# wushan270/mit-6.824-2015

Hardware: AMD Instinct MI355X
Metric: word-count input GB/s (whole node) and % of HBM roofline at 1/2/4/8 MI355X (higher is better)
Workload: dtype u8

## Files before the change

mit-6.824-2015_amd/csrc/wcg_agg.h:

```cpp
#pragma once
#include "wcg_common.h"
#include "wcg_lds_table.h"
#include "wcg_map.h"

namespace wcg {

constexpr int AGG_NT = 1024;
constexpr u32 AGG_BATCH = AGG_NT * 4;
constexpr int AGG_W = 2;
constexpr int AGG_NB = 3350;
constexpr u32 AGG_SLACK_UNITS = AGG_BATCH + 8;
constexpr u32 AGG_MAX_SRC = 256;
constexpr u32 AGG_Q = 128;
constexpr u32 AGG_OVF_CAP = 4096;
constexpr int AGG_SPILL = 0, AGG_EMIT = 1;
#ifndef WCG_AGG_PROBES
#define WCG_AGG_PROBES 2
#endif
constexpr int AGG_PROBES = WCG_AGG_PROBES;
#ifndef WCG_AGG_SPEC_K1
#define WCG_AGG_SPEC_K1 0
#endif
constexpr bool AGG_SPEC_K1 = WCG_AGG_SPEC_K1;
#ifndef WCG_AGG_SPEC_MED
#define WCG_AGG_SPEC_MED 1
#endif
#ifndef WCG_AGG_KINDS
#define WCG_AGG_KINDS 1
#endif
#ifndef WCG_AGG_ABLATE
#define WCG_AGG_ABLATE 0
#endif

struct AggArgs {
    const u64* pool;
    const u32* region_len;
    u64 region_cap;
    u32 P;
    u32 nsrc;
    u32 slices;
    u32 pm;
    u32 slices_m;
    u32 nbi;
    u32 ls_nreg;
    u32 rstride, rmod;
    u32 P1;
    int mode;
    GEntry* gtab;
    u64 gmask;
    DevState* st;
    const u64* map_stats;
    u64* spill;
    u64 spill_cap;
    u32* spill_len;
    Rec* emit;
    u64 emit_cap;
    Rec* ovf;
    u32 ovf_cap;
    u64* clk;
    uint16_t* flist;
};

#ifndef WCG_AGG2_LDSHASH
#define WCG_AGG2_LDSHASH 0
#endif
__device__ __forceinline__ u32 agg_hash(u64 k0, u64 k1) {
    if (WCG_AGG2_LDSHASH) return lds_hash(k0, k1) * 0x9E3779B1u;
    return (u32)(key_hash(k0, k1) >> 32);
}

__device__ __forceinline__ void agg_decode(const u64 (&u)[6], u64 (&k0)[4], u64 (&k1)[4], u64 (&c)[4], bool (&v)[4],
                                           u32 (&nu)[4]) {
#pragma unroll
    for (int k = 0; k < 4; k++) {
        const u32 T = (u32)(u[k] >> 56);
        const bool head = T >= 0x41;
        v[k] = T != 0 && (head || (T & 0x1F) < 8);
        const u64 last = head ? u[k + 1] : u[k];
        k0[k] = head ? u[k] : (u[k] & ~U_CNT);
        k1[k] = head ? (u[k + 1] & ~U_CNT) : 0;
        const bool hc = (last & U_CNT) != 0;
        c[k] = hc ? (head ? u[k + 2] : u[k + 1]) : 1;
        nu[k] = (head ? 2u : 1u) + (hc ? 1u : 0u);
    }
}

__device__ __forceinline__ void agg_decode_short(const u64 (&u)[6], u64 (&k0)[4], u64 (&k1)[4], u64 (&c)[4], bool (&v)[4],
                                                 u32 (&nu)[4]) {
#pragma unroll
    for (int k = 0; k < 4; k++) {
        v[k] = (u[k] >> 56) != 0;
        const bool hc = (u[k] & U_CNT) != 0;
        k0[k] = u[k] & ~U_CNT;
        k1[k] = 0;
        c[k] = hc ? u[k + 1] : 1;
        nu[k] = hc ? 2u : 1u;
    }
}
__device__ __forceinline__ void agg_decode_medium(const u64 (&u)[6], u64 (&k0)[4], u64 (&k1)[4], u64 (&c)[4], bool (&v)[4],
                                                  u32 (&nu)[4]) {
#pragma unroll
    for (int k = 0; k < 4; k++) {
        v[k] = (u32)(u[k] >> 56) >= 0x41;
        const bool hc = (u[k + 1] & U_CNT) != 0;
        k0[k] = u[k];
        k1[k] = u[k + 1] & ~U_CNT;
        c[k] = hc ? u[k + 2] : 1;
        nu[k] = hc ? 3u : 2u;
    }
}

#define WCG_AGG_SET_OPS(S)                                                                      \
    __device__ __forceinline__ void agg_load_##S(const v4u* q, v4u& x0, v4u& x1, v4u& x2) {     \
        asm volatile("global_load_dwordx4 %0, %3, off ; wcg-load " #S "0\n\t"                   \
                     "global_load_dwordx4 %1, %3, off offset:16 ; wcg-load " #S "1\n\t"         \
                     "global_load_dwordx4 %2, %3, off offset:32 ; wcg-load " #S "2"              \
                     : "=&v"(x0), "=&v"(x1), "=&v"(x2) : "v"(q) : "memory");                    \
    }                                                                                           \
    template <int N>                                                                            \
    __device__ __forceinline__ void agg_wait_##S(v4u& x0, v4u& x1, v4u& x2) {                   \
        asm volatile("s_waitcnt vmcnt(%3) ; wcg-wait " #S " %0 %1 %2"                            \
                     : "+v"(x0), "+v"(x1), "+v"(x2) : "n"(N) : "memory");                       \
    }
WCG_AGG_SET_OPS(A)
WCG_AGG_SET_OPS(B)
WCG_AGG_SET_OPS(C)
#undef WCG_AGG_SET_OPS
#ifndef WCG_AGG_SETS1
#define WCG_AGG_SETS1 2
#endif
#ifndef WCG_AGG_SETS2
#define WCG_AGG_SETS2 2
#endif

template <int MODE, int KIND>
__device__ __forceinline__ u64 agg_one(const AggArgs& a, u32 bi, u64 (*tk0)[AGG_W], u64 (*tk1)[AGG_W], u64 (*tcnt)[AGG_W], u32* rlen_s,
                       u32* bstart, u32& spos, u64 (*wsum)[4]) {
    const int tid = threadIdx.x;
    LdsTable<AGG_NB, u64, AGG_W> tab{tk0, tk1, tcnt};
    constexpr bool emit = MODE == AGG_EMIT;
    u32 p, s, sl;
    if (bi < a.pm * a.slices) { p = bi % a.pm; s = bi / a.pm; sl = a.slices; }
    else { const u32 b2 = bi - a.pm * a.slices, nm = a.P - a.pm; p = a.pm + b2 % nm; s = b2 / nm; sl = a.slices_m; }
#ifdef WCG_AGG_MREV
    if (p >= a.pm && a.pm < a.P) p = a.P - 1 - (p - a.pm);
#endif
    u32 k0_, k1_, wbase, wstep;
    if (!emit) {
        k0_ = (u32)(((u64)a.nsrc * s) / sl); k1_ = (u32)(((u64)a.nsrc * (s + 1)) / sl);
        wbase = 0; wstep = 1;
    } else {
        k0_ = 0; k1_ = a.nsrc;
        wbase = p / AGG_Q; wstep = a.P1;
    }
    const u32 nk = k1_ - k0_;
    auto region = [&](u32 k) -> u64 { return (u64)(wbase + k * wstep) * a.rstride + p % a.rmod; };
    constexpr u32 WB = 256;
    for (u32 k = tid; k < nk; k += AGG_NT) rlen_s[k] = a.region_len[region(k0_ + k)];
    __syncthreads();
    if (tid == 0) {
        u32 t = 0;
        for (u32 k = 0; k < nk; k++) { bstart[k] = t; t += (rlen_s[k] + WB - 1) / WB; }
        bstart[nk] = t;
        spos = 0;
    }
    __syncthreads();
    const u32 nbat = bstart[nk];
    if (nbat == 0) {
        if (!emit && tid == 0 && a.spill_len) a.spill_len[bi] = 0;
        return 0;
    }
    tab.init(tid, AGG_NT);
    __syncthreads();
    u64 my_global = 0;
    u64* const sp = emit ? nullptr : a.spill + (u64)bi * a.spill_cap;
    auto overflow = [&](u64 k0, u64 k1, u64 c, u32 nu) {
        if (emit) {
            const u32 pos = atomicAdd(&spos, 1u);
            if (pos < a.ovf_cap) { a.ovf[(u64)blockIdx.x * a.ovf_cap + pos] = inline_rec(k0, k1, c); return; }
        } else {
            const u32 pos = atomicAdd(&spos, nu);
            if (pos + nu <= a.spill_cap) {
                u64 e[3];
                const u64 f = c > 1 ? U_CNT : 0;
                if (key_short(k0)) { e[0] = k0 | f; e[1] = c; }
                else { e[0] = k0; e[1] = k1 | f; e[2] = c; }
                for (u32 j = 0; j < nu; j++) sp[pos + j] = e[j];
                return;
            }
            for (u64 j = pos; j < a.spill_cap; j++) sp[j] = 0;
        }
        my_global++;
        ginsert(a.gtab, a.gmask, k0, k1, gslot(key_hash(k0, k1)), c, a.st);
    };
    const u32 wave = (u32)__builtin_amdgcn_readfirstlane(tid >> 6), lane = tid & 63;
    constexpr u32 WSTRIDE = AGG_NT / 64;
    const bool per_wave = !emit;
    auto advance = [&](u32& k, u32& b, u32 step) {
        if (per_wave) {
            b += step / WSTRIDE;
            while (k < nk && b >= bstart[k + 1] - bstart[k]) { k += WSTRIDE; b = 0; }
            return;
        }
        b += step;
        while (k < nk) {
            const u32 nbk = bstart[k + 1] - bstart[k];
            if (b < nbk) break;
            b -= nbk;
            k++;
        }
    };
    auto batch_ptr = [&](u32 k, u32 b) -> const v4u* {
        const bool live = k < nk;
        const u64 i = (live ? (u64)b * WB : 0) + 4 * lane;
        return reinterpret_cast<const v4u*>(a.pool + region(k0_ + (live ? k : 0)) * a.region_cap + i);
    };
    auto unit = [](const v4u& x, int h) -> u64 { return h ? ((u64)x.w << 32 | x.z) : ((u64)x.y << 32 | x.x); };
    auto process = [&](u32 k, u32 b, const v4u& x0, const v4u& x1, const v4u& x2) {
        u64 u[6] = {unit(x0, 0), unit(x0, 1), unit(x1, 0), unit(x1, 1), unit(x2, 0), unit(x2, 1)};
        const u32 i0 = b * WB + 4 * lane, len = rlen_s[k];
#pragma unroll
        for (int j = 0; j < 6; j++) u[j] = i0 + j < len ? u[j] : 0;
        if (WCG_AGG_ABLATE == 1) { asm volatile("" ::"v"(u[0] ^ u[1] ^ u[2] ^ u[3] ^ u[4] ^ u[5])); return; }
        u64 k0[4], k1[4], c[4];
        bool v[4];
        u32 nu[4];
        if (KIND == 1) agg_decode_short(u, k0, k1, c, v, nu);
        else if (KIND == 2) agg_decode_medium(u, k0, k1, c, v, nu);
        else agg_decode(u, k0, k1, c, v, nu);
        if (WCG_AGG_ABLATE == 4) {
#pragma unroll
            for (int j = 0; j < 4; j++) v[j] = v[j] && key_short(k0[j]);
        }
        if (WCG_AGG_ABLATE == 2) {
            u32 x = 0;
#pragma unroll
            for (int j = 0; j < 4; j++) x ^= v[j] ? lds_hash(k0[j], k1[j]) + (u32)c[j] : 0u;
            asm volatile("" ::"v"(x));
            return;
        }
        static_assert(4 % AGG_PROBES == 0, "probe groups split a lane's 4 units");
        constexpr bool SPEC = KIND == 2 ? WCG_AGG_SPEC_MED : AGG_SPEC_K1;
#pragma unroll
        for (int j = 0; j < 4; j += AGG_PROBES) {
            typename decltype(tab)::Probe pr[AGG_PROBES];
#pragma unroll
            for (int q = 0; q < AGG_PROBES; q++) {
                const u32 h = emit ? agg_hash(k0[j + q], k1[j + q]) : lds_hash(k0[j + q], k1[j + q]);
                if (!v[j + q]) continue;
                if (SPEC) tab.start_k1(h, KIND == 2 || !key_short(k0[j + q]), pr[q]);
                else tab.start(h, pr[q]);
            }
#pragma unroll
            for (int q = 0; q < AGG_PROBES; q++) {
                if (!v[j + q]) continue;
                const bool ok = SPEC ? tab.template finish_k1<KIND>(k0[j + q], k1[j + q], pr[q], c[j + q])
                                     : tab.template finish<KIND>(k0[j + q], k1[j + q], pr[q], c[j + q]);
                if (!ok) overflow(k0[j + q], k1[j + q], c[j + q], nu[j + q]);
            }
        }
    };
    constexpr int NSETS = emit ? WCG_AGG_SETS2 : WCG_AGG_SETS1;
    static_assert(NSETS == 2 || NSETS == 3, "k_agg's batch walk names two or three register sets");
    u32 kA = 0, bA = 0, kB, bB, kC = 0, bC = 0;
    if (per_wave) { kA = wave; bA = (u32)-1; advance(kA, bA, WSTRIDE); }
    else advance(kA, bA, wave);
    kB = kA; bB = bA;
    advance(kB, bB, WSTRIDE);
    v4u a0, a1, a2, b0, b1, b2, c0, c1, c2;
    agg_load_A(batch_ptr(kA, bA), a0, a1, a2);
    agg_load_B(batch_ptr(kB, bB), b0, b1, b2);
    if (NSETS == 3) {
        kC = kB; bC = bB;
        advance(kC, bC, WSTRIDE);
        agg_load_C(batch_ptr(kC, bC), c0, c1, c2);
        while (kA < nk) {
            agg_wait_A<6>(a0, a1, a2);
            process(kA, bA, a0, a1, a2);
            kA = kC; bA = bC;
            advance(kA, bA, WSTRIDE);
            agg_load_A(batch_ptr(kA, bA), a0, a1, a2);
            if (kB >= nk) break;
            agg_wait_B<6>(b0, b1, b2);
            process(kB, bB, b0, b1, b2);
            kB = kA; bB = bA;
            advance(kB, bB, WSTRIDE);
            agg_load_B(batch_ptr(kB, bB), b0, b1, b2);
            if (kC >= nk) break;
            agg_wait_C<6>(c0, c1, c2);
            process(kC, bC, c0, c1, c2);
            kC = kB; bC = bB;
            advance(kC, bC, WSTRIDE);
            agg_load_C(batch_ptr(kC, bC), c0, c1, c2);
        }
        agg_wait_C<0>(c0, c1, c2);
    } else {
        while (kA < nk) {
            agg_wait_A<3>(a0, a1, a2);
            process(kA, bA, a0, a1, a2);
            kA = kB; bA = bB;
            advance(kA, bA, WSTRIDE);
            agg_load_A(batch_ptr(kA, bA), a0, a1, a2);
            if (kB >= nk) break;
            agg_wait_B<3>(b0, b1, b2);
            process(kB, bB, b0, b1, b2);
            kB = kA; bB = bA;
            advance(kB, bB, WSTRIDE);
            agg_load_B(batch_ptr(kB, bB), b0, b1, b2);
        }
    }
    agg_wait_A<0>(a0, a1, a2);
    agg_wait_B<0>(b0, b1, b2);
    __syncthreads();
    if (!emit && a.flist && !a.spill_cap && WCG_AGG_ABLATE != 3) {
        constexpr u32 NE = AGG_NB * AGG_W;
        uint16_t* const L = a.flist + (u64)bi * NE;
        u32 mine = 0;
        for (int i = tid; i < (int)NE; i += AGG_NT) mine += (&tcnt[0][0])[i] ? 1u : 0u;
        u32 incl = mine;
        for (int d = 1; d < 64; d <<= 1) { const u32 y = __shfl_up(incl, d, 64); if (lane >= (u32)d) incl += y; }
        if (lane == 63) wsum[wave][0] = incl;
        __syncthreads();
        u32 pos = 0, all = 0;
        for (u32 w = 0; w < AGG_NT / 64; w++) { if (w < wave) pos += (u32)wsum[w][0]; all += (u32)wsum[w][0]; }
        pos += incl - mine;
        for (int i = tid; i < (int)NE; i += AGG_NT)
            if ((&tcnt[0][0])[i]) L[pos++] = (uint16_t)i;
        asm volatile("s_waitcnt vmcnt(0)" ::: "memory");
        __syncthreads();
        for (u32 j = tid; j < all; j += AGG_NT) {
            const u32 i = __hip_atomic_load(&L[j], __ATOMIC_RELAXED, __HIP_MEMORY_SCOPE_AGENT);
            const u64 c = (&tcnt[0][0])[i], k0 = (&tk0[0][0])[i], k1 = (&tk1[0][0])[i];
            my_global++;
            ginsert(a.gtab, a.gmask, k0, k1, gslot(key_hash(k0, k1)), c, a.st);
        }
        __syncthreads();
    } else if (!emit) {
        for (int i = tid; i < AGG_NB * AGG_W; i += AGG_NT) {
            const u64 c = (&tcnt[0][0])[i];
            if (!c || WCG_AGG_ABLATE == 3) continue;
            const u64 k0 = (&tk0[0][0])[i], k1 = (&tk1[0][0])[i];
            if (a.spill_cap) { overflow(k0, k1, c, (u32)entry_units(k0, (u32)(c > 1 ? 2 : 1))); continue; }
            my_global++;
            ginsert(a.gtab, a.gmask, k0, k1, gslot(key_hash(k0, k1)), c, a.st);
        }
        __syncthreads();
        if (tid == 0 && a.spill_len) a.spill_len[bi] = spos < a.spill_cap ? spos : (u32)a.spill_cap;
    } else {
        u32 mine = 0;
        for (int i = tid; i < AGG_NB * AGG_W; i += AGG_NT) mine += (&tcnt[0][0])[i] ? 1u : 0u;
        u32 incl = mine;
        for (int d = 1; d < 64; d <<= 1) { const u32 y = __shfl_up(incl, d, 64); if (lane >= d) incl += y; }
        if (lane == 63) wsum[wave][0] = incl;
        __syncthreads();
        u32 pre = 0, all = 0;
        for (int w = 0; w < AGG_NT / 64; w++) { if (w < wave) pre += (u32)wsum[w][0]; all += (u32)wsum[w][0]; }
        const u32 nov = spos < a.ovf_cap ? spos : a.ovf_cap;
        if (tid == 0)
            wsum[0][1] = all + nov ? atomicAdd((unsigned long long*)&a.st->nemit, (unsigned long long)(all + nov)) : 0;
        __syncthreads();
        const u64 base = wsum[0][1];
        for (u32 i = tid; i < nov; i += AGG_NT) {
            const Rec r = a.ovf[(u64)blockIdx.x * a.ovf_cap + i];
            if (base + all + i < a.emit_cap) a.emit[base + all + i] = r;
            else {
                my_global++;
                u64 k0, k1;
                rec_inline_key(r, k0, k1);
                ginsert(a.gtab, a.gmask, k0, k1, gslot(key_hash(k0, k1)), r.cnt, a.st);
            }
        }
        u64 pos = base + pre + incl - mine;
        for (int i = tid; i < AGG_NB * AGG_W; i += AGG_NT) {
            const u64 c = (&tcnt[0][0])[i];
            if (!c) continue;
            const u64 k0 = (&tk0[0][0])[i], k1 = (&tk1[0][0])[i];
            if (pos < a.emit_cap) a.emit[pos] = inline_rec(k0, k1, c);
            else { my_global++; ginsert(a.gtab, a.gmask, k0, k1, gslot(key_hash(k0, k1)), c, a.st); }
            pos++;
        }
    }
    __syncthreads();
    return my_global;
}

struct AggTabs {
    u64 tk0[AGG_NB][AGG_W];
    u64 tk1[AGG_NB][AGG_W];
    u64 tcnt[AGG_NB][AGG_W];
};
union AggLds {
    AggTabs t;
    LsLds ls;
};
static_assert(LS_NT == AGG_NT, "long_small runs as a k_agg workgroup");
template <int MODE>
__global__ __launch_bounds__(AGG_NT) void k_agg(AggArgs a, MapArgs ma) {
    __shared__ __align__(16) AggLds lds;
    u64 (*const tk0)[AGG_W] = lds.t.tk0;
    u64 (*const tk1)[AGG_W] = lds.t.tk1;
    u64 (*const tcnt)[AGG_W] = lds.t.tcnt;
    __shared__ u32 rlen_s[AGG_MAX_SRC];
    __shared__ u32 bstart[AGG_MAX_SRC + 1];
    __shared__ u32 spos;
    __shared__ u64 wsum[AGG_NT / 64][4];
    const int tid = threadIdx.x;
    const u32 nb = a.nbi;
    if (MODE == AGG_SPILL && a.ls_nreg && blockIdx.x == nb) {
        long_small(ma, a.ls_nreg, lds.ls);
        return;
    }
    const u64 t0 = a.clk ? wall_clock64() : 0;
    if (MODE == AGG_SPILL && blockIdx.x == 0 && tid == 0) { a.st->nrec = 0; a.st->nlong = 0; }
    u64 my_global = 0;
    for (u32 bi = blockIdx.x; bi < nb; bi += gridDim.x)
        if (MODE == AGG_SPILL && WCG_AGG_KINDS && a.pm < a.P)
            my_global += bi < a.pm * a.slices ? agg_one<MODE, 1>(a, bi, tk0, tk1, tcnt, rlen_s, bstart, spos, wsum)
                                              : agg_one<MODE, 2>(a, bi, tk0, tk1, tcnt, rlen_s, bstart, spos, wsum);
        else
            my_global += agg_one<MODE, 0>(a, bi, tk0, tk1, tcnt, rlen_s, bstart, spos, wsum);
    for (int d = 32; d >= 1; d >>= 1) my_global += __shfl_xor(my_global, d, 64);
    u64 ms = 0;
    if (blockIdx.x == 0 && MODE != AGG_EMIT)
        for (u32 w = tid >> 2; w < a.nsrc; w += AGG_NT / 4) ms += a.map_stats[(u64)w * 4 + (tid & 3)];
    for (int d = 32; d >= 4; d >>= 1) ms += __shfl_xor(ms, d, 64);
    if ((tid & 63) < 4) wsum[tid >> 6][tid & 3] = ms + ((tid & 63) == 2 ? my_global : 0);
    __syncthreads();
    if (tid < 4) {
        u64 t = 0;
        for (int w = 0; w < AGG_NT / 64; w++) t += wsum[w][tid];
        u64* dst[4] = {&a.st->tokens, &a.st->lds_hits, &a.st->global_ops, &a.st->long_tokens};
        if (t) atomicAdd(dst[tid], t);
    }
    if (a.clk && tid == 0) { a.clk[2 * blockIdx.x] = t0; a.clk[2 * blockIdx.x + 1] = wall_clock64(); }
}

#ifndef WCG_RP_QB
#define WCG_RP_QB 48
#endif
#ifndef WCG_RP_PREFETCH
#define WCG_RP_PREFETCH 0
#endif
constexpr u32 RP_QB = WCG_RP_QB;
struct RpArgs {
    const u64* pool; const u32* region_len; u64 region_cap;
    u32 P, nsrc, slices;
    const u64* map_stats;
    u64* pool2; u64 cap2; u32* region_len2;
    GEntry* gtab; u64 gmask; DevState* st;
};
#ifndef WCG_RP_MINB
#define WCG_RP_MINB 1
#endif
__global__ __launch_bounds__(AGG_NT, WCG_RP_MINB) void k_rp(RpArgs a) {
    __shared__ u64 sbuf[AGG_Q][RP_QB];
    __shared__ u32 scnt[AGG_Q], sfill[AGG_Q], gpos[AGG_Q], gbase[AGG_Q];
    __shared__ u32 sdirect[AGG_Q];
    __shared__ u64 wsum[AGG_NT / 64][4];
    const u32 b = blockIdx.x, tid = threadIdx.x;
    const u32 p = b % a.P, sl = b / a.P;
    const u32 k0_ = (u32)(((u64)a.nsrc * sl) / a.slices), k1_ = (u32)(((u64)a.nsrc * (sl + 1)) / a.slices);
    u64* const pool2 = a.pool2;
    const u64 cap2 = a.cap2;
    GEntry* const gtab = a.gtab;
    const u64 gmask = a.gmask;
    DevState* const st = a.st;
    if (b == 0) {
        u64 ms = 0;
        for (u32 w = tid >> 2; w < a.nsrc; w += AGG_NT / 4) ms += a.map_stats[(u64)w * 4 + (tid & 3)];
        for (int d = 32; d >= 4; d >>= 1) ms += __shfl_xor(ms, d, 64);
        if ((tid & 63) < 4) wsum[tid >> 6][tid & 3] = ms;
        __syncthreads();
        if (tid < 4) {
            u64 t = 0;
            for (int w = 0; w < AGG_NT / 64; w++) t += wsum[w][tid];
            u64* dst4[4] = {&st->tokens, &st->lds_hits, &st->global_ops, &st->long_tokens};
            if (t) atomicAdd(dst4[tid], t);
        }
    }
    for (u32 q = tid; q < AGG_Q; q += AGG_NT) { scnt[q] = 0; sfill[q] = 0; gpos[q] = 0; }
    __syncthreads();
    u64* const dst = pool2 + (u64)b * AGG_Q * cap2;
    u64 my_global = 0;
    auto encode = [](u64 k0, u64 k1, u64 c, u64 (&e)[3]) {
        const u64 f = c > 1 ? U_CNT : 0;
        if (key_short(k0)) { e[0] = k0 | f; e[1] = c; }
        else { e[0] = k0; e[1] = k1 | f; e[2] = c; }
    };
    auto to_region = [&](u32 q, u64 pos, const u64 (&e)[3], u32 nu, u64 k0, u64 k1, u64 c) {
        u64* r = dst + (u64)q * cap2;
        if (pos + nu <= cap2) { for (u32 t = 0; t < nu; t++) r[pos + t] = e[t]; return; }
        for (u64 t = pos; t < cap2; t++) r[t] = 0;
        my_global++;
        ginsert(gtab, gmask, k0, k1, gslot(key_hash(k0, k1)), c, st);
    };
#if WCG_RP_PREFETCH
    u32 k = k0_, base = 0, n = k < k1_ ? a.region_len[(u64)k * a.P + p] : 0u;
    while (k < k1_ && n == 0) { k++; n = k < k1_ ? a.region_len[(u64)k * a.P + p] : 0u; }
    u64 nu[6];
    auto load6 = [&](u32 kk, u32 bb, u32 nn, u64 (&x)[6]) {
        const u64* s = a.pool + ((u64)kk * a.P + p) * a.region_cap;
        const u32 i = bb + 4 * tid;
#pragma unroll
        for (int j = 0; j < 6; j++) x[j] = kk < k1_ && i + j < nn ? s[i + j] : 0;
    };
    load6(k, 0, n, nu);
    while (k < k1_) {
        u64 u[6];
#pragma unroll
        for (int j = 0; j < 6; j++) u[j] = nu[j];
        u32 kn = k, bn = base + AGG_BATCH, nn = n;
        if (bn >= n) {
            bn = 0;
            do { kn++; nn = kn < k1_ ? a.region_len[(u64)kn * a.P + p] : 0u; } while (kn < k1_ && nn == 0);
        }
        load6(kn, bn, nn, nu);
        {
#else
    for (u32 k = k0_; k < k1_; k++) {
    const u64 reg = (u64)k * a.P + p;
    const u32 n = a.region_len[reg];
    const u64* src = a.pool + reg * a.region_cap;
    for (u32 base = 0; base < n; base += AGG_BATCH) {
        const u32 i0 = base + 4 * tid;
        u64 u[6];
#pragma unroll
        for (int j = 0; j < 6; j++) u[j] = i0 + j < n ? src[i0 + j] : 0;
#endif
        u64 k0[4], k1[4], c[4];
        bool v[4];
        u32 nu[4];
        agg_decode(u, k0, k1, c, v, nu);
#pragma unroll
        for (int j = 0; j < 4; j++) {
            if (!v[j]) continue;
            const u32 q = (u32)(key_hash(k0[j], k1[j]) >> 40) & (AGG_Q - 1);
            u64 e[3];
            encode(k0[j], k1[j], c[j], e);
            const u32 pos = atomicAdd(&scnt[q], nu[j]);
            if (pos + nu[j] <= RP_QB) {
                for (u32 t = 0; t < nu[j]; t++) sbuf[q][pos + t] = e[t];
                atomicMax(&sfill[q], pos + nu[j]);
            } else {
                to_region(q, atomicAdd(&gpos[q], nu[j]), e, nu[j], k0[j], k1[j], c[j]);
            }
        }
        __syncthreads();
        for (u32 q = tid; q < AGG_Q; q += AGG_NT) {
            gbase[q] = gpos[q];
            gpos[q] += sfill[q];
            sdirect[q] = (u64)gbase[q] + sfill[q] > cap2;
        }
        __syncthreads();
        for (u32 t = tid; t < AGG_Q * RP_QB; t += AGG_NT) {
            const u32 q = t / RP_QB, j = t % RP_QB;
            if (j < sfill[q] && !sdirect[q]) dst[(u64)q * cap2 + gbase[q] + j] = sbuf[q][j];
        }
        for (u32 q = tid; q < AGG_Q; q += AGG_NT) {
            if (!sdirect[q]) continue;
            u64 pos = gbase[q];
            for (u32 j = 0; j < sfill[q];) {
                u64 y[6] = {sbuf[q][j], j + 1 < sfill[q] ? sbuf[q][j + 1] : 0, j + 2 < sfill[q] ? sbuf[q][j + 2] : 0, 0, 0, 0};
                u64 kk0[4], kk1[4], cc[4];
                bool vv[4];
                u32 nn[4];
                agg_decode(y, kk0, kk1, cc, vv, nn);
                u64 e[3];
                encode(kk0[0], kk1[0], cc[0], e);
                to_region(q, pos, e, nn[0], kk0[0], kk1[0], cc[0]);
                pos += nn[0];
                j += nn[0];
            }
        }
        __syncthreads();
        for (u32 q = tid; q < AGG_Q; q += AGG_NT) { scnt[q] = 0; sfill[q] = 0; }
        __syncthreads();
    }
#if WCG_RP_PREFETCH
        k = kn; base = bn; n = nn;
#endif
    }
    for (u32 q = tid; q < AGG_Q; q += AGG_NT) a.region_len2[(u64)b * AGG_Q + q] = gpos[q] < cap2 ? gpos[q] : (u32)cap2;
    for (int d = 32; d >= 1; d >>= 1) my_global += __shfl_xor(my_global, d, 64);
    if ((tid & 63) == 0 && my_global) atomicAdd(&st->global_ops, my_global);
}

}
```

mit-6.824-2015_amd/csrc/wcg_lds_table.h:

```cpp
#pragma once
#include "wcg_common.h"
#ifndef WCG_DIAG_SLOTS
#define WCG_DIAG_SLOTS 0
#endif
#ifndef WCG_MAP_ROW2
#define WCG_MAP_ROW2 0
#endif
#ifndef WCG_DIAG_NOCOUNT
#define WCG_DIAG_NOCOUNT 0
#endif

namespace wcg {

template <int NB, typename CNT, int W>
struct LdsTable {
    static_assert(W == 2 || W == 4, "rows of one or two 16-byte reads");
    u64 (*k0)[W];
    u64 (*k1)[W];
    CNT (*cnt)[W];

    struct Probe {
        u32 b1, b2;
        u64 v[W], w[W];
        u64 v1[W], w1[W];
    };

    __device__ __forceinline__ void init(int tid, int nt) {
        for (int i = tid; i < NB * W; i += nt) {
            (&k0[0][0])[i] = 0;
            (&k1[0][0])[i] = 0;
            (&cnt[0][0])[i] = 0;
        }
    }

    __device__ __forceinline__ static void buckets(u32 h, u32& b1, u32& b2) {
        b1 = __umulhi(h, (u32)NB);
        u32 m = h * 0x85EBCA6Bu;
        m ^= m >> 15;
        b2 = __umulhi(m * 0xC2B2AE35u, (u32)NB);
        if (b2 == b1) b2 = (b1 + 1 == (u32)NB) ? 0 : b1 + 1;
    }

    __device__ __forceinline__ void readrow(u32 b, u64 (&v)[W]) const {
        const uint4* p = reinterpret_cast<const uint4*>(&k0[b][0]);
#pragma unroll
        for (int q = 0; q < W / 2; q++) {
            const uint4 x = p[q];
            v[2 * q] = (u64)x.y << 32 | x.x;
            v[2 * q + 1] = (u64)x.w << 32 | x.z;
        }
    }

    __device__ __forceinline__ void start(u32 h, Probe& p) const {
        buckets(h, p.b1, p.b2);
        readrow(p.b1, p.v);
        readrow(p.b2, p.w);
    }

    __device__ __forceinline__ void start_k1(u32 h, bool med, Probe& p) const {
        buckets(h, p.b1, p.b2);
        readrow(p.b1, p.v);
        readrow(p.b2, p.w);
        if (med) {
            const uint4* q1 = reinterpret_cast<const uint4*>(&k1[p.b1][0]);
            const uint4* q2 = reinterpret_cast<const uint4*>(&k1[p.b2][0]);
#pragma unroll
            for (int q = 0; q < W / 2; q++) {
                const uint4 x = q1[q], y = q2[q];
                p.v1[2 * q] = (u64)x.y << 32 | x.x; p.v1[2 * q + 1] = (u64)x.w << 32 | x.z;
                p.w1[2 * q] = (u64)y.y << 32 | y.x; p.w1[2 * q + 1] = (u64)y.w << 32 | y.z;
            }
        } else {
#pragma unroll
            for (int j = 0; j < W; j++) { p.v1[j] = 0; p.w1[j] = 0; }
        }
    }

    __device__ __forceinline__ void add_cnt(u32 b, int j, CNT c) { atomicAdd(&cnt[b][j], c); }

    template <int KIND = 0>
    __device__ __forceinline__ bool finish_k1(u64 a0, u64 a1, const Probe& p, CNT c) {
        u32 m = 0;
#pragma unroll
        for (int j = 0; j < W; j++) {
            m |= (u32)(p.v[j] == a0 && p.v1[j] == a1) << j;
            m |= (u32)(p.w[j] == a0 && p.w1[j] == a1) << (W + j);
        }
        if (m) {
            const int s = __ffs(m) - 1;
            add_cnt(s < W ? p.b1 : p.b2, s % W, c);
            return true;
        }
        return finish<KIND>(a0, a1, p, c);
    }

    template <int KIND = 0>
    __device__ __forceinline__ bool finish(u64 a0, u64 a1, const Probe& p, CNT c) {
        const bool shrt = KIND == 1 ? true : KIND == 2 ? false : key_short(a0);
        u32 m = 0, e = 0;
#pragma unroll
        for (int j = 0; j < W; j++) {
            m |= (u32)(p.v[j] == a0) << j;
            m |= (u32)(p.w[j] == a0) << (W + j);
            e |= (u32)(p.v[j] == 0) << j;
            e |= (u32)(p.w[j] == 0) << (W + j);
        }
        if (!shrt && m) {
            u32 mm = m;
            m = 0;
            while (mm) {
                const int s = __ffs(mm) - 1;
                mm &= mm - 1;
                if (k1[s < W ? p.b1 : p.b2][s % W] == a1) { m = 1u << s; break; }
            }
        }
        if (m) {
            const int s = __ffs(m) - 1;
            add_cnt(s < W ? p.b1 : p.b2, s % W, c);
            return true;
        }
        const u32 e1 = e & ((1u << W) - 1), e2 = e >> W;
        const bool second = __popc(e2) > __popc(e1);
        auto try_bucket = [&](u32 b, u32 m) -> bool {
            while (m) {
                const int j = __ffs(m) - 1;
                m &= m - 1;
                const u64 old = atomicCAS(&k0[b][j], 0ull, a0);
                if (old == 0) {
                    if (!shrt) k1[b][j] = a1;
                    add_cnt(b, j, c);
                    return true;
                }
                if (old == a0 && (shrt || k1[b][j] == a1)) { add_cnt(b, j, c); return true; }
            }
            return false;
        };
        if (second) return try_bucket(p.b2, e2) || try_bucket(p.b1, e1);
        return try_bucket(p.b1, e1) || try_bucket(p.b2, e2);
    }

    __device__ __forceinline__ bool add(u64 a0, u64 a1, u32 h, CNT c) {
        Probe p;
        start(h, p);
        return finish(a0, a1, p, c);
    }
};

template <int NS, int NM>
struct MapTable {
    u64* sk0;
    u32* scnt;
    u64* mk0;
    u64* mk1;
    u32* mcnt;
    u64* zero;
    u32* seen;

    __device__ __forceinline__ void init(int tid, int nt) {
        for (int i = tid; i < NS; i += nt) { sk0[i] = 0; scnt[i] = 0; }
        for (int i = tid; i < NM; i += nt) { mk0[i] = 0; mk1[i] = 0; mcnt[i] = 0; }
        if (seen) for (int i = tid; i < (int)(ADMIT_BITS / 32); i += nt) seen[i] = 0;
        if (tid == 0) *zero = 0;
    }
    static constexpr u32 ADMIT_BITS = 16384;
    __device__ __forceinline__ bool admit(u32 h) {
        if (!seen) return true;
        const u32 b = (h * 0x9E3779B1u) >> 18;
        const u32 bit = 1u << (b & 31);
        return (atomicOr(&seen[b >> 5], bit) & bit) != 0;
    }
    __device__ __forceinline__ static void slots(u32 h, u32 n, u32& s1, u32& s2) {
#if WCG_DIAG_SLOTS
        s1 = __lane_id(); s2 = __lane_id() + 64; (void)h; (void)n;
#else
        s1 = (u32)(((u64)(h >> 8) * (u64)(n << 8)) >> 32);
        s2 = (u32)(((u64)(h & 0xFFFFFFu) * (u64)(n << 8)) >> 32);
#endif
    }
    struct Probe { u32 s1, s2; u64 x1, x2, y1, y2; };
    __device__ __forceinline__ Probe probe(bool med, u32 h) const {
        static_assert(NS < 65536 && NM < 65536, "n << 8 fits the 24-bit multiply");
        Probe p;
        slots(h, med ? (u32)NM : (u32)NS, p.s1, p.s2);
        const u64* K0 = med ? mk0 : sk0;
        p.x1 = K0[p.s1]; p.x2 = K0[p.s2];
        const u64* K1a = med ? mk1 + p.s1 : zero;
        const u64* K1b = med ? mk1 + p.s2 : zero;
        p.y1 = *K1a; p.y2 = *K1b;
        return p;
    }
    struct ProbeS { u32 s1, s2; u64 x1, x2; };
    __device__ __forceinline__ ProbeS probe_short(u32 h) const {
        ProbeS p;
#if WCG_MAP_ROW2
        static_assert(NS % 2 == 0, "rows of two short slots");
        p.s1 = 2 * (u32)(((u64)(h >> 8) * (u64)((NS / 2) << 8)) >> 32);
        p.s2 = p.s1 + 1;
        const uint4 r = *reinterpret_cast<const uint4*>(sk0 + p.s1);
        p.x1 = (u64)r.y << 32 | r.x; p.x2 = (u64)r.w << 32 | r.z;
#else
        slots(h, (u32)NS, p.s1, p.s2);
        p.x1 = sk0[p.s1]; p.x2 = sk0[p.s2];
#endif
        return p;
    }
    __device__ __forceinline__ bool finish_short(u64 a0, u32 h, const ProbeS& p) {
        const bool h1 = p.x1 == a0, hit = h1 || p.x2 == a0;
        if (!WCG_DIAG_NOCOUNT) atomicAdd(&scnt[h1 ? p.s1 : p.s2], hit ? 1u : 0u);
        if (hit || (p.x1 != 0 && p.x2 != 0) || !admit(h)) return hit;
        if (p.x1 == 0) {
            const u64 old = atomicCAS(&sk0[p.s1], 0ull, a0);
            if (old == 0 || old == a0) { atomicAdd(&scnt[p.s1], 1u); return true; }
        }
        if (p.x2 == 0) {
            const u64 old = atomicCAS(&sk0[p.s2], 0ull, a0);
            if (old == 0 || old == a0) { atomicAdd(&scnt[p.s2], 1u); return true; }
        }
        return false;
    }

    __device__ __forceinline__ bool finish_short_v(bool valid, u64 a0, u32 h, const ProbeS& p) {
        const bool h1 = p.x1 == a0, hit = valid && (h1 || p.x2 == a0);
        atomicAdd(&scnt[h1 ? p.s1 : p.s2], hit ? 1u : 0u);
        if (!valid || hit || (p.x1 != 0 && p.x2 != 0) || !admit(h)) return hit;
        if (p.x1 == 0) {
            const u64 old = atomicCAS(&sk0[p.s1], 0ull, a0);
            if (old == 0 || old == a0) { atomicAdd(&scnt[p.s1], 1u); return true; }
        }
        if (p.x2 == 0) {
            const u64 old = atomicCAS(&sk0[p.s2], 0ull, a0);
            if (old == 0 || old == a0) { atomicAdd(&scnt[p.s2], 1u); return true; }
        }
        return false;
    }

    __device__ __forceinline__ bool finish(bool valid, bool med, u64 a0, u64 a1, u32 h, const Probe& p) {
        u64* K0 = med ? mk0 : sk0;
        u32* C = med ? mcnt : scnt;
        const bool h1 = p.x1 == a0 && p.y1 == a1, h2 = p.x2 == a0 && p.y2 == a1;
        const bool hit = valid && (h1 || h2);
        atomicAdd(&C[h1 ? p.s1 : p.s2], hit ? 1u : 0u);
        if (!valid || hit || (p.x1 != 0 && p.x2 != 0) || !admit(h)) return hit;
        if (p.x1 == 0) {
            const u64 old = atomicCAS(&K0[p.s1], 0ull, a0);
            if (old == 0) {
                if (med) mk1[p.s1] = a1;
                atomicAdd(&C[p.s1], 1u);
                return true;
            }
            if (old == a0 && !med) { atomicAdd(&C[p.s1], 1u); return true; }
        }
        if (p.x2 == 0) {
            const u64 old = atomicCAS(&K0[p.s2], 0ull, a0);
            if (old == 0) {
                if (med) mk1[p.s2] = a1;
                atomicAdd(&C[p.s2], 1u);
                return true;
            }
            if (old == a0 && !med) { atomicAdd(&C[p.s2], 1u); return true; }
        }
        return false;
    }
};

__device__ __forceinline__ u32 miss_bucket(u32 h, u32 pmask) { return h & pmask; }
__device__ __forceinline__ u64 gslot(u64 h2) { return h2 >> 16; }

constexpr u64 U_CNT = 1ull << 61;

__device__ __forceinline__ int entry_units(u64 k0, u32 c) { return (key_short(k0) ? 1 : 2) + (c > 1 ? 1 : 0); }

__device__ __forceinline__ void put_entry(u64* u, u64 k0, u64 k1, u32 c) {
    const u64 f = c > 1 ? U_CNT : 0;
    if (key_short(k0)) {
        u[0] = k0 | f;
        if (c > 1) u[1] = c;
    } else {
        u[0] = k0;
        u[1] = k1 | f;
        if (c > 1) u[2] = c;
    }
}

}
```

Measured before the change: 1159.

## Straight-line branchless hit path and 24-bit bucket hash in LDS aggregation

Adds a branchless finish_hit path for short-key aggregation. Every lane probes and issues an atomicAdd, with zero added for invalid or missing units, so that lanes do not diverge on the validity check. Masked-out tail units get distinct dummy keys instead of zero. Bucket selection switches to a cheaper 24-bit multiply scheme (buckets24), and new flags are added for last-batch masking and an even per-wave split (both off by default). The cost is extra LDS atomics that add zero, and a different bucket distribution that may change collision and overflow rates.

```diff
diff --git a/mit-6.824-2015_amd/csrc/wcg_agg.h b/mit-6.824-2015_amd/csrc/wcg_agg.h
--- a/mit-6.824-2015_amd/csrc/wcg_agg.h
+++ b/mit-6.824-2015_amd/csrc/wcg_agg.h
@@ -27,6 +27,18 @@
 #endif
 #ifndef WCG_AGG_KINDS
 #define WCG_AGG_KINDS 1
+#endif
+#ifndef WCG_AGG_LASTMASK
+#define WCG_AGG_LASTMASK 0
+#endif
+#ifndef WCG_AGG_STRAIGHT
+#define WCG_AGG_STRAIGHT 1
+#endif
+#ifndef WCG_AGG_HASH24
+#define WCG_AGG_HASH24 1
+#endif
+#ifndef WCG_AGG_EVEN
+#define WCG_AGG_EVEN 0
 #endif
 #ifndef WCG_AGG_ABLATE
 #define WCG_AGG_ABLATE 0
@@ -196,13 +208,16 @@
     const u32 wave = (u32)__builtin_amdgcn_readfirstlane(tid >> 6), lane = tid & 63;
     constexpr u32 WSTRIDE = AGG_NT / 64;
     const bool per_wave = !emit;
+    const u32 nk16 = WCG_AGG_EVEN && per_wave ? nk - nk % WSTRIDE : nk;
     auto advance = [&](u32& k, u32& b, u32 step) {
-        if (per_wave) {
+        if (per_wave && k < nk16) {
             b += step / WSTRIDE;
-            while (k < nk && b >= bstart[k + 1] - bstart[k]) { k += WSTRIDE; b = 0; }
-            return;
-        }
-        b += step;
+            while (k < nk16 && b >= bstart[k + 1] - bstart[k]) { k += WSTRIDE; b = 0; }
+            if (k < nk16) return;
+            k = nk16; b = wave;
+        } else {
+            b += step;
+        }
         while (k < nk) {
             const u32 nbk = bstart[k + 1] - bstart[k];
             if (b < nbk) break;
@@ -218,9 +233,14 @@
     auto unit = [](const v4u& x, int h) -> u64 { return h ? ((u64)x.w << 32 | x.z) : ((u64)x.y << 32 | x.x); };
     auto process = [&](u32 k, u32 b, const v4u& x0, const v4u& x1, const v4u& x2) {
         u64 u[6] = {unit(x0, 0), unit(x0, 1), unit(x1, 0), unit(x1, 1), unit(x2, 0), unit(x2, 1)};
+        constexpr bool SPEC = KIND == 2 ? WCG_AGG_SPEC_MED : AGG_SPEC_K1;
+        constexpr bool SL = !emit && ((KIND == 1 && !SPEC && (WCG_AGG_STRAIGHT & 1)) || (KIND == 2 && SPEC && (WCG_AGG_STRAIGHT & 2)));
+        constexpr bool B24 = !emit && (KIND == 1 ? (WCG_AGG_HASH24 & 1) != 0 : KIND == 2 ? (WCG_AGG_HASH24 & 2) != 0 : false);
         const u32 i0 = b * WB + 4 * lane, len = rlen_s[k];
-#pragma unroll
-        for (int j = 0; j < 6; j++) u[j] = i0 + j < len ? u[j] : 0;
+        if (!(WCG_AGG_LASTMASK && !emit && KIND != 0) || (b + 1) * WB + 2 > len) {
+#pragma unroll
+            for (int j = 0; j < 6; j++) u[j] = i0 + j < len ? u[j] : (SL ? (u64)(i0 + j) : 0);
+        }
         if (WCG_AGG_ABLATE == 1) { asm volatile("" ::"v"(u[0] ^ u[1] ^ u[2] ^ u[3] ^ u[4] ^ u[5])); return; }
         u64 k0[4], k1[4], c[4];
         bool v[4];
@@ -240,21 +260,21 @@
             return;
         }
         static_assert(4 % AGG_PROBES == 0, "probe groups split a lane's 4 units");
-        constexpr bool SPEC = KIND == 2 ? WCG_AGG_SPEC_MED : AGG_SPEC_K1;
 #pragma unroll
         for (int j = 0; j < 4; j += AGG_PROBES) {
             typename decltype(tab)::Probe pr[AGG_PROBES];
 #pragma unroll
             for (int q = 0; q < AGG_PROBES; q++) {
                 const u32 h = emit ? agg_hash(k0[j + q], k1[j + q]) : lds_hash(k0[j + q], k1[j + q]);
-                if (!v[j + q]) continue;
-                if (SPEC) tab.start_k1(h, KIND == 2 || !key_short(k0[j + q]), pr[q]);
-                else tab.start(h, pr[q]);
+                if (!SL && !v[j + q]) continue;
+                if (SPEC) tab.template start_k1<B24>(h, KIND == 2 || !key_short(k0[j + q]), pr[q]);
+                else tab.template start<B24>(h, pr[q]);
             }
 #pragma unroll
             for (int q = 0; q < AGG_PROBES; q++) {
-                if (!v[j + q]) continue;
-                const bool ok = SPEC ? tab.template finish_k1<KIND>(k0[j + q], k1[j + q], pr[q], c[j + q])
+                if (!SL && !v[j + q]) continue;
+                const bool ok = SL ? tab.template finish_hit<(KIND ? KIND : 1)>(v[j + q], k0[j + q], k1[j + q], pr[q], c[j + q])
+                                : SPEC ? tab.template finish_k1<KIND>(k0[j + q], k1[j + q], pr[q], c[j + q])
                                      : tab.template finish<KIND>(k0[j + q], k1[j + q], pr[q], c[j + q]);
                 if (!ok) overflow(k0[j + q], k1[j + q], c[j + q], nu[j + q]);
             }
@@ -263,7 +283,7 @@
     constexpr int NSETS = emit ? WCG_AGG_SETS2 : WCG_AGG_SETS1;
     static_assert(NSETS == 2 || NSETS == 3, "k_agg's batch walk names two or three register sets");
     u32 kA = 0, bA = 0, kB, bB, kC = 0, bC = 0;
-    if (per_wave) { kA = wave; bA = (u32)-1; advance(kA, bA, WSTRIDE); }
+    if (per_wave && nk16) { kA = wave; bA = (u32)-1; advance(kA, bA, WSTRIDE); }
     else advance(kA, bA, wave);
     kB = kA; bB = bA;
     advance(kB, bB, WSTRIDE);
diff --git a/mit-6.824-2015_amd/csrc/wcg_lds_table.h b/mit-6.824-2015_amd/csrc/wcg_lds_table.h
--- a/mit-6.824-2015_amd/csrc/wcg_lds_table.h
+++ b/mit-6.824-2015_amd/csrc/wcg_lds_table.h
@@ -41,6 +41,13 @@
         if (b2 == b1) b2 = (b1 + 1 == (u32)NB) ? 0 : b1 + 1;
     }
 
+    __device__ __forceinline__ static void buckets24(u32 h, u32& b1, u32& b2) {
+        static_assert(NB < 65536, "NB << 8 fits the 24-bit multiply");
+        b1 = (u32)(((u64)(h >> 8) * (u64)((u32)NB << 8)) >> 32);
+        b2 = (u32)(((u64)(h & 0xFFFFFFu) * (u64)((u32)(NB - 1) << 8)) >> 32);
+        b2 += b2 >= b1 ? 1u : 0u;
+    }
+
     __device__ __forceinline__ void readrow(u32 b, u64 (&v)[W]) const {
         const uint4* p = reinterpret_cast<const uint4*>(&k0[b][0]);
 #pragma unroll
@@ -51,14 +58,18 @@
         }
     }
 
+    template <bool B24 = false>
     __device__ __forceinline__ void start(u32 h, Probe& p) const {
-        buckets(h, p.b1, p.b2);
+        if (B24) buckets24(h, p.b1, p.b2);
+        else buckets(h, p.b1, p.b2);
         readrow(p.b1, p.v);
         readrow(p.b2, p.w);
     }
 
+    template <bool B24 = false>
     __device__ __forceinline__ void start_k1(u32 h, bool med, Probe& p) const {
-        buckets(h, p.b1, p.b2);
+        if (B24) buckets24(h, p.b1, p.b2);
+        else buckets(h, p.b1, p.b2);
         readrow(p.b1, p.v);
         readrow(p.b2, p.w);
         if (med) {
@@ -92,6 +103,25 @@
             return true;
         }
         return finish<KIND>(a0, a1, p, c);
+    }
+
+    template <int KIND>
+    __device__ __forceinline__ bool finish_hit(bool valid, u64 a0, u64 a1, const Probe& p, CNT c) {
+        static_assert(KIND == 1 || KIND == 2, "one kind of key per bucket");
+        bool in1 = false, in2 = false;
+        u32 j1 = W - 1, j2 = W - 1;
+#pragma unroll
+        for (int j = W - 1; j >= 0; j--) {
+            const bool x = p.v[j] == a0 && (KIND == 1 || p.v1[j] == a1);
+            const bool y = p.w[j] == a0 && (KIND == 1 || p.w1[j] == a1);
+            in1 = in1 || x; j1 = x ? (u32)j : j1;
+            in2 = in2 || y; j2 = y ? (u32)j : j2;
+        }
+        const bool hit = valid && (in1 || in2);
+        const u32 slot = in1 ? p.b1 * W + j1 : p.b2 * W + j2;
+        atomicAdd(&(&cnt[0][0])[slot], hit ? c : (CNT)0);
+        if (valid && !hit) return finish<KIND>(a0, a1, p, c);
+        return true;
     }
 
     template <int KIND = 0>
```

Result: no change. 1163 (median of 6 runs) (+0.3%).
